# kubeai-project/kubeai

Hardware: AMD Instinct MI355X
Metric: output_tokens_per_s (k6 multi-turn chat) (higher is better)
Workload: dtype fp8; 1 GPU; model=llama-3-8b, global_batch=40, seq_len=8192, parallelism=dp1, prefix_cache=True

## Files before the change

kubeai_amd/csrc/attention_decode.hip:

```cpp
#include <torch/extension.h>

#include <type_traits>

#include "attention_checks.h"
#include "attention_plan.h"
#include "common.h"
#include "dispatch.h"

namespace {

constexpr int kWaves = 2;
constexpr int kBlockThreads = kWaves * WAVE_SIZE;
constexpr int kBS = 16;
typedef __attribute__((ext_vector_type(2))) __bf16 bf16x2v;
constexpr int kPad = 8;

template <int G, typename CT = ushort, int HD = 128, bool CAP = false,
          bool RAW = false>
__launch_bounds__(kBlockThreads) __global__ void paged_decode_kernel(
    ushort* __restrict__ out,
    const ushort* __restrict__ q,
    std::conditional_t<RAW, CT*, const CT*> __restrict__ k_cache,
    std::conditional_t<RAW, CT*, const CT*> __restrict__ v_cache,
    const int32_t* __restrict__ block_tables,
// ... 299 lines not shown
      }

#pragma unroll
      for (int t = tp; t < tp + TOKP; ++t) {
        if (t >= tile_len) break;
        float vv[EPL];
        if constexpr (sizeof(CT) == 2) {
#pragma unroll
          for (int e = 0; e < EPL; e += 2) {
            const uint32_t vr = *reinterpret_cast<const uint32_t*>(
                &v_lds[wave][t][EPL * lane + e]);
            vv[e] = bf16_to_f32((ushort)(vr & 0xffff));
            vv[e + 1] = bf16_to_f32((ushort)(vr >> 16));
          }
        } else {
#pragma unroll
          for (int e = 0; e < EPL; e += 2) {
            const uint32_t vr = *reinterpret_cast<const ushort*>(
                &v_lds[wave][t][EPL * lane + e]);
            const floatx2 vf = __builtin_amdgcn_cvt_pk_f32_bf8(vr, false);
            vv[e] = vf.x;
            vv[e + 1] = vf.y;
          }
        }
#pragma unroll
        for (int g = 0; g < G; ++g) {
          const float pt = __shfl(p[g], (t - tp) * PARTS, 64);
#pragma unroll
          for (int e = 0; e < EPL; ++e)
            o[g][e] = fmaf(pt, vv[e], o[g][e]);
        }
      }
    }

    if (blk_i + kWaves < blk_hi) write_tile();
  }

#pragma unroll
  for (int g = 0; g < G; ++g) {
#pragma unroll
    for (int e = 0; e < EPL; ++e) merge_o[wave][g][EPL * lane + e] = o[g][e];
    if (lane == 0) {
      merge_ml[wave][g][0] = m[g];
      merge_ml[wave][g][1] = l[g];
    }
  }
  __syncthreads();

  for (int g = wave; g < G; g += kWaves) {
    float m_star = -INFINITY;
#pragma unroll
    for (int w = 0; w < kWaves; ++w) m_star = fmaxf(m_star, merge_ml[w][g][0]);
    float l_star = 0.f, oo[EPL];
#pragma unroll
    for (int e = 0; e < EPL; ++e) oo[e] = 0.f;
    if (m_star != -INFINITY) {
#pragma unroll
      for (int w = 0; w < kWaves; ++w) {
        const float c = __expf(merge_ml[w][g][0] - m_star);
        l_star += merge_ml[w][g][1] * c;
#pragma unroll
        for (int e = 0; e < EPL; ++e)
          oo[e] += merge_o[w][g][EPL * lane + e] * c;
      }
    }
    const int head = kh * G + g;
    if (n_splits == 1) {
      const float inv_l = 1.0f / l_star;
      ushort* oh = out + ((int64_t)b * n_q + head) * HD;
#pragma unroll
      for (int e = 0; e < EPL; e += 2) {
        uint32_t packed =
            ((uint32_t)f32_to_bf16(oo[e + 1] * inv_l) << 16) |
            f32_to_bf16(oo[e] * inv_l);
        *reinterpret_cast<uint32_t*>(&oh[EPL * lane + e]) = packed;
      }
    } else {
      float* po = part_o + (((int64_t)b * n_q + head) * n_splits + split) * HD;
#pragma unroll
      for (int e = 0; e < EPL; ++e) po[EPL * lane + e] = oo[e];
      if (lane == 0) {
        float* pm = part_ml + (((int64_t)b * n_q + head) * n_splits + split) * 2;
        pm[0] = m_star;
        pm[1] = l_star;
      }
    }
  }
}

constexpr int kMergeSplitCapLo = 8;
constexpr int kMergeSplitCapHi = 16;

template <int N, int HD, int SCAP>
DEV_INLINE void merge_partials(const float* __restrict__ po,
                               const float* __restrict__ pml,
                               const int n_splits, uint32_t (&packed)[N / 2]) {
  typedef float __attribute__((ext_vector_type(N))) vecN;
  floatx2 ml[SCAP];
  vecN pv[SCAP];
#pragma unroll
  for (int s = 0; s < SCAP; ++s) {
    const int sc = min(s, n_splits - 1);
    ml[s] = *reinterpret_cast<const floatx2*>(pml + 2 * sc);
    pv[s] = *reinterpret_cast<const vecN*>(po + sc * HD);
  }
  __builtin_amdgcn_sched_barrier(0);
  float m_star = -INFINITY;
#pragma unroll
  for (int s = 0; s < SCAP; ++s)
    if (s < n_splits) m_star = fmaxf(m_star, ml[s].x);
  float l_star = 0.f, oo[N];
#pragma unroll
  for (int e = 0; e < N; ++e) oo[e] = 0.f;
#pragma unroll
  for (int s = 0; s < SCAP; ++s) {
    const bool use = s < n_splits && ml[s].x != -INFINITY;
    const float c = __expf(ml[s].x - m_star);
    l_star = use ? l_star + ml[s].y * c : l_star;
#pragma unroll
    for (int e = 0; e < N; ++e) oo[e] = use ? oo[e] + pv[s][e] * c : oo[e];
  }
  const float inv_l = 1.0f / l_star;
#pragma unroll
  for (int e = 0; e < N; e += 2)
    packed[e / 2] = ((uint32_t)f32_to_bf16(oo[e + 1] * inv_l) << 16) |
                    f32_to_bf16(oo[e] * inv_l);
}

template <int HD, int SCAP>
__global__ void decode_merge_kernel(
    ushort* __restrict__ out,
    const float* __restrict__ part_o,
    const float* __restrict__ part_ml,
    const int n_q, const int n_splits, const int64_t n_bh) {
  constexpr int EPL = HD / 64;
  const int64_t bh = (int64_t)blockIdx.x * (blockDim.x / WAVE_SIZE) +
                     threadIdx.x / WAVE_SIZE;
  if (bh >= n_bh) return;
  const int lane = threadIdx.x % WAVE_SIZE;
  uint32_t packed[EPL / 2];
  merge_partials<EPL, HD, SCAP>(part_o + bh * n_splits * HD + EPL * lane,
                                part_ml + bh * n_splits * 2, n_splits, packed);
  ushort* oh = out + bh * HD;
#pragma unroll
  for (int e = 0; e < EPL; e += 2)
    *reinterpret_cast<uint32_t*>(&oh[EPL * lane + e]) = packed[e / 2];
}

constexpr int kMergeVec = 4;
constexpr int kMergeMaxThreads = 1024;
constexpr int kMergeMaxPasses = 2;
constexpr int kMergeRowMax = kMergeMaxThreads * kMergeVec * kMergeMaxPasses;

template <int HD, int kPasses, int SCAP>
__launch_bounds__(kMergeMaxThreads) __global__ void decode_merge_fp8_kernel(
    ushort* __restrict__ out,
    unsigned char* __restrict__ out_fp8,
    float* __restrict__ out_scale,
    const float* __restrict__ part_o,
    const float* __restrict__ part_ml,
    const int n_q, const int n_splits) {
  __shared__ float red[16];
  const int b = blockIdx.x;
  const int row_len = n_q * HD;
  const int nvec = row_len / kMergeVec;
  ushort* orow = out + (int64_t)b * row_len;

  uint32_t packed[kPasses][kMergeVec / 2];
  float amax = 0.f;
#pragma unroll
  for (int it = 0; it < kPasses; ++it) {
    const int i = threadIdx.x + it * blockDim.x;
    if (i < nvec) {
      const int h = (i * kMergeVec) / HD;
      const int col = (i * kMergeVec) % HD;
      const int64_t bh = (int64_t)b * n_q + h;
      merge_partials<kMergeVec, HD, SCAP>(part_o + bh * n_splits * HD + col,
                                          part_ml + bh * n_splits * 2,
                                          n_splits, packed[it]);
      *reinterpret_cast<uint2*>(orow + i * kMergeVec) =
          make_uint2(packed[it][0], packed[it][1]);
#pragma unroll
      for (int e = 0; e < kMergeVec / 2; ++e) {
        const uint32_t pk = packed[it][e];
        amax = fmaxf(amax, fabsf(bf16_to_f32((ushort)(pk & 0xffff))));
        amax = fmaxf(amax, fabsf(bf16_to_f32((ushort)(pk >> 16))));
      }
    }
  }
  const float inv_scale = row_scale_fp8(amax, red, out_scale + b);
  unsigned char* frow = out_fp8 + (int64_t)b * row_len;
#pragma unroll
  for (int it = 0; it < kPasses; ++it) {
    const int i = threadIdx.x + it * blockDim.x;
    if (i < nvec) {
      uchar4 q4;
      const uint32_t p0 = packed[it][0], p1 = packed[it][1];
      q4.x = f32_to_fp8(bf16_to_f32((ushort)(p0 & 0xffff)) * inv_scale);
      q4.y = f32_to_fp8(bf16_to_f32((ushort)(p0 >> 16)) * inv_scale);
      q4.z = f32_to_fp8(bf16_to_f32((ushort)(p1 & 0xffff)) * inv_scale);
      q4.w = f32_to_fp8(bf16_to_f32((ushort)(p1 >> 16)) * inv_scale);
      *reinterpret_cast<uchar4*>(frow + i * kMergeVec) = q4;
    }
  }
}

}

void quant_fp8(torch::Tensor out, torch::Tensor out_scale, torch::Tensor x);

namespace {

struct RawQKV {
  torch::Tensor k, v, positions, cos_sin, slot_mapping;
};

void decode_impl(torch::Tensor out, const c10::optional<torch::Tensor>& out_fp8,
                 const c10::optional<torch::Tensor>& out_scale, torch::Tensor q,
                 torch::Tensor k_cache, torch::Tensor v_cache,
                 torch::Tensor block_tables, torch::Tensor seq_lens,
                 double scale, int64_t window, double softcap,
                 const RawQKV* raw = nullptr) {
  const AttnShape s =
      check_paged_attention(out, q, k_cache, v_cache, block_tables, seq_lens);
  const int B = q.size(0), n_q = s.n_q, n_kv = s.n_kv, hd = s.hd;
  const int max_blocks = s.max_blocks;
  TORCH_CHECK(seq_lens.numel() >= B && block_tables.size(0) >= B);
  const bool want_fp8 = out_fp8.has_value();
  if (want_fp8) {
    TORCH_CHECK(out_scale.has_value());
    check_fp8_out(out, *out_fp8, *out_scale);
  }
  const ushort *k_new = nullptr, *v_new = nullptr;
  const int32_t* positions = nullptr;
  const float* cos_sin = nullptr;
  const int64_t* slot_mapping = nullptr;
  int64_t k_stride = 0, v_stride = 0;
  if (raw != nullptr) {
    const torch::Tensor &k = raw->k, &v = raw->v;
    TORCH_CHECK(k.dim() == 3 && v.dim() == 3);
    TORCH_CHECK(k.scalar_type() == torch::kBFloat16 &&
                v.scalar_type() == torch::kBFloat16);
    TORCH_CHECK(k.size(0) == B && k.size(1) == n_kv && k.size(2) == hd);
    TORCH_CHECK(v.size(0) == B && v.size(1) == n_kv && v.size(2) == hd);
    TORCH_CHECK(k.stride(2) == 1 && k.stride(1) == hd);
    TORCH_CHECK(v.stride(2) == 1 && v.stride(1) == hd);
    TORCH_CHECK(v_cache.sizes() == k_cache.sizes() &&
                v_cache.scalar_type() == k_cache.scalar_type());
    TORCH_CHECK(k_cache.size(3) == hd);
    TORCH_CHECK(raw->positions.scalar_type() == torch::kInt32 &&
                raw->positions.is_contiguous() && raw->positions.numel() >= B);
    TORCH_CHECK(raw->slot_mapping.scalar_type() == torch::kInt64 &&
                raw->slot_mapping.is_contiguous() &&
                raw->slot_mapping.numel() >= B);
    TORCH_CHECK(raw->cos_sin.scalar_type() == torch::kFloat32 &&
                raw->cos_sin.dim() == 2 && raw->cos_sin.size(1) == hd &&
                raw->cos_sin.is_contiguous());
    auto aligned = [](const torch::Tensor& t, int64_t bytes) {
      return reinterpret_cast<uintptr_t>(t.data_ptr()) % bytes == 0 &&
             (t.dim() < 3 || t.stride(0) * t.element_size() % bytes == 0);
    };
    TORCH_CHECK(aligned(q, 8) && aligned(k, 16) && aligned(v, 16) &&
                    aligned(raw->cos_sin, 16) && aligned(k_cache, 16) &&
                    aligned(v_cache, 16),
                "rope_cache_attention_decode: misaligned q/k/v/cos_sin/cache");
    k_new = (const ushort*)k.data_ptr();
    v_new = (const ushort*)v.data_ptr();
    positions = raw->positions.data_ptr<int32_t>();
    cos_sin = raw->cos_sin.data_ptr<float>();
    slot_mapping = raw->slot_mapping.data_ptr<int64_t>();
    k_stride = k.stride(0);
    v_stride = v.stride(0);
  }
  if (B == 0) return;
  const int n_splits = attn_plan::decode_n_splits(B, n_kv, max_blocks);
  torch::Tensor part_o, part_ml;
  float *part_o_ptr = nullptr, *part_ml_ptr = nullptr;
  if (n_splits > 1) {
    auto opts =
        torch::TensorOptions().device(q.device()).dtype(torch::kFloat32);
    part_o = torch::empty({B, n_q, n_splits, (int64_t)hd}, opts);
    part_ml = torch::empty({B, n_q, n_splits, 2}, opts);
    part_o_ptr = part_o.data_ptr<float>();
    part_ml_ptr = part_ml.data_ptr<float>();
  }
  dim3 grid(B * n_kv * n_splits), block(kBlockThreads);
  auto stream = c10::hip::getCurrentHIPStream().stream();
  dispatch_int<1, 2, 4, 5, 6, 8>(s.G, "GQA group size", [&](auto g) {
    dispatch_int<128, 256>(hd, "head dim", [&](auto hdv) {
      dispatch_bool(s.fp8_cache, [&](auto fp8) {
        dispatch_bool(softcap > 0.0, [&](auto cap) {
          dispatch_bool(raw != nullptr, [&](auto rawv) {
            using CT = std::conditional_t<decltype(fp8)::value, unsigned char,
                                          ushort>;
            hipLaunchKernelGGL(
                (paged_decode_kernel<decltype(g)::value, CT,
                                     decltype(hdv)::value, decltype(cap)::value,
                                     decltype(rawv)::value>),
                grid, block, 0, stream, (ushort*)out.data_ptr(),
                (const ushort*)q.data_ptr(), (CT*)k_cache.data_ptr(),
                (CT*)v_cache.data_ptr(), block_tables.data_ptr<int32_t>(),
                seq_lens.data_ptr<int32_t>(), (float)scale, (float)softcap,
                (int)window, n_kv, max_blocks, q.stride(0), n_splits,
                part_o_ptr, part_ml_ptr, k_new, v_new, positions, cos_sin,
                slot_mapping, k_stride, v_stride);
          });
        });
      });
    });
  });
  HIP_CHECK_KERNEL();
  if (n_splits == 1) {
    if (want_fp8) quant_fp8(*out_fp8, *out_scale, out.view({B, -1}));
    return;
  }
  static_assert(kMergeSplitCapHi == 16, "decode_n_splits caps splits at 16");
  TORCH_CHECK(n_splits <= kMergeSplitCapHi);
  const bool fuse_fp8 = want_fp8 && (int64_t)n_q * hd <= kMergeRowMax;
  dispatch_int<128, 256>(hd, "head dim", [&](auto hdv) {
    dispatch_bool(n_splits <= kMergeSplitCapLo, [&](auto lo) {
      constexpr int HD = decltype(hdv)::value;
      constexpr int SCAP =
          decltype(lo)::value ? kMergeSplitCapLo : kMergeSplitCapHi;
      if (fuse_fp8) {
        const int nvec = n_q * hd / kMergeVec;
        const int threads = std::min(
            kMergeMaxThreads, (nvec + WAVE_SIZE - 1) / WAVE_SIZE * WAVE_SIZE);
        dispatch_int<1, 2>(
            (nvec + threads - 1) / threads, "merge pass count", [&](auto p) {
              hipLaunchKernelGGL(
                  (decode_merge_fp8_kernel<HD, decltype(p)::value, SCAP>),
                  dim3(B), dim3(threads), 0, stream, (ushort*)out.data_ptr(),
                  (unsigned char*)out_fp8->data_ptr(),
                  out_scale->data_ptr<float>(), part_o_ptr, part_ml_ptr, n_q,
                  n_splits);
            });
      } else {
        const int64_t n_bh = (int64_t)B * n_q;
        const int wpb = 4;
        hipLaunchKernelGGL((decode_merge_kernel<HD, SCAP>),
                           dim3((uint32_t)((n_bh + wpb - 1) / wpb)),
                           dim3(wpb * WAVE_SIZE), 0, stream,
                           (ushort*)out.data_ptr(), part_o_ptr, part_ml_ptr,
                           n_q, n_splits, n_bh);
      }
    });
  });
  HIP_CHECK_KERNEL();
  if (want_fp8 && !fuse_fp8) quant_fp8(*out_fp8, *out_scale, out.view({B, -1}));
}

}

void paged_attention_decode(torch::Tensor out, torch::Tensor q,
                            torch::Tensor k_cache, torch::Tensor v_cache,
                            torch::Tensor block_tables, torch::Tensor seq_lens,
                            double scale, int64_t window, double softcap) {
  decode_impl(out, c10::nullopt, c10::nullopt, q, k_cache, v_cache,
              block_tables, seq_lens, scale, window, softcap);
}

void paged_attention_decode_fp8(torch::Tensor out, torch::Tensor out_fp8,
                                torch::Tensor out_scale, torch::Tensor q,
                                torch::Tensor k_cache, torch::Tensor v_cache,
                                torch::Tensor block_tables,
                                torch::Tensor seq_lens, double scale,
                                int64_t window, double softcap) {
  decode_impl(out, out_fp8, out_scale, q, k_cache, v_cache, block_tables,
              seq_lens, scale, window, softcap);
}

void rope_cache_attention_decode(
    torch::Tensor out, c10::optional<torch::Tensor> out_fp8,
    c10::optional<torch::Tensor> out_scale, torch::Tensor q, torch::Tensor k,
    torch::Tensor v, torch::Tensor positions, torch::Tensor cos_sin,
    torch::Tensor k_cache, torch::Tensor v_cache, torch::Tensor slot_mapping,
    torch::Tensor block_tables, torch::Tensor seq_lens, double scale,
    int64_t window, double softcap) {
  const RawQKV raw{k, v, positions, cos_sin, slot_mapping};
  decode_impl(out, out_fp8, out_scale, q, k_cache, v_cache, block_tables,
              seq_lens, scale, window, softcap, &raw);
}
```

kubeai_amd/csrc/bindings.cpp:

```cpp
#include <torch/extension.h>

#include <utility>

#include "attention_plan.h"

void rmsnorm(torch::Tensor out, torch::Tensor x, torch::Tensor weight,
             double eps);
void fused_add_rmsnorm(torch::Tensor x, torch::Tensor residual,
                       torch::Tensor weight, double eps);
void rope(torch::Tensor q, torch::Tensor k, torch::Tensor positions,
          torch::Tensor cos_sin);
void rope_and_cache(torch::Tensor q, torch::Tensor k, torch::Tensor v,
                    torch::Tensor positions, torch::Tensor cos_sin,
                    torch::Tensor k_cache, torch::Tensor v_cache,
                    torch::Tensor slot_mapping);
void reshape_and_cache(torch::Tensor k, torch::Tensor v, torch::Tensor k_cache,
                       torch::Tensor v_cache, torch::Tensor slot_mapping);
void paged_attention_decode(torch::Tensor out, torch::Tensor q,
                            torch::Tensor k_cache, torch::Tensor v_cache,
                            torch::Tensor block_tables, torch::Tensor seq_lens,
                            double scale, int64_t window, double softcap);
void paged_attention_decode_fp8(torch::Tensor out, torch::Tensor out_fp8,
                                torch::Tensor out_scale, torch::Tensor q,
                                torch::Tensor k_cache, torch::Tensor v_cache,
                                torch::Tensor block_tables,
                                torch::Tensor seq_lens, double scale,
                                int64_t window, double softcap);
void rope_cache_attention_decode(
    torch::Tensor out, c10::optional<torch::Tensor> out_fp8,
    c10::optional<torch::Tensor> out_scale, torch::Tensor q, torch::Tensor k,
    torch::Tensor v, torch::Tensor positions, torch::Tensor cos_sin,
    torch::Tensor k_cache, torch::Tensor v_cache, torch::Tensor slot_mapping,
    torch::Tensor block_tables, torch::Tensor seq_lens, double scale,
    int64_t window, double softcap);
void paged_attention_prefill(torch::Tensor out, torch::Tensor q,
                             torch::Tensor k_cache, torch::Tensor v_cache,
                             torch::Tensor block_tables,
                             torch::Tensor query_start_loc,
                             torch::Tensor seq_lens, double scale,
                             int64_t window, double softcap);
void silu_and_mul(torch::Tensor out, torch::Tensor x);
void gelu_and_mul(torch::Tensor out, torch::Tensor x);
void skinny_gemm(torch::Tensor y, torch::Tensor x, torch::Tensor w);
void int4_dequant(torch::Tensor out, torch::Tensor qp, torch::Tensor sp,
                  torch::Tensor zp, int64_t N, int64_t K, int64_t group);
void int4_gemm(torch::Tensor y, torch::Tensor x, torch::Tensor qp,
               torch::Tensor sp, torch::Tensor zp, int64_t N, int64_t K,
               int64_t group);
int64_t int4_gemm_tiles(int64_t N, int64_t M);
void greedy_sample(torch::Tensor out, torch::Tensor logits);
void gumbel_sample(torch::Tensor out, torch::Tensor logits,
                   torch::Tensor temperature, torch::Tensor seeds,
                   int64_t step);
void greedy_sample_logprob(torch::Tensor out, torch::Tensor out_logprob,
                           torch::Tensor out_lse, torch::Tensor logits);
void gumbel_sample_logprob(torch::Tensor out, torch::Tensor out_logprob,
                           torch::Tensor out_lse, torch::Tensor logits,
                           torch::Tensor temperature, torch::Tensor seeds,
                           int64_t step);
void token_logprobs(torch::Tensor out_logprob, torch::Tensor out_lse,
                    torch::Tensor logits, torch::Tensor tokens);
void sgmv(torch::Tensor y, torch::Tensor x, torch::Tensor A, torch::Tensor B,
          torch::Tensor idx, double scale);
void register_chwbl(pybind11::module_& m);
pybind11::bytes xgmi_alloc();
void xgmi_connect(int64_t rank, int64_t world,
                  const std::vector<pybind11::bytes>& handles);
void xgmi_fused_allreduce_add_rmsnorm(torch::Tensor x, torch::Tensor residual,
                                      torch::Tensor weight, double eps);
int64_t xgmi_error_count();
int64_t xgmi_max_elems();
void xgmi_shutdown();
void rmsnorm_fp8(torch::Tensor out, torch::Tensor out_scale, torch::Tensor x,
                 torch::Tensor weight, double eps);
void fused_add_rmsnorm_fp8(torch::Tensor out, torch::Tensor out_scale,
                           torch::Tensor x, torch::Tensor residual,
                           torch::Tensor weight, double eps);
void fused_add_rmsnorm_fp8_div(torch::Tensor out, torch::Tensor out_scale,
                               torch::Tensor x, torch::Tensor residual,
                               torch::Tensor weight, double eps,
                               bool write_rows);
void embed_rmsnorm_fp8(torch::Tensor out, torch::Tensor out_scale,
                       torch::Tensor x_out, torch::Tensor ids,
                       torch::Tensor table, torch::Tensor weight, double eps);
void silu_and_mul_fp8(torch::Tensor out, torch::Tensor out_scale,
                      torch::Tensor x);
void quant_fp8(torch::Tensor out, torch::Tensor out_scale, torch::Tensor x);
void quant_fp8_div(torch::Tensor out, torch::Tensor out_scale,
                   torch::Tensor x);
void nucleus_stats(torch::Tensor m, torch::Tensor z, torch::Tensor logits,
                   torch::Tensor temps);
void nucleus_accept(torch::Tensor ok, torch::Tensor logits,
                    torch::Tensor cand, torch::Tensor m, torch::Tensor z,
                    torch::Tensor temps, torch::Tensor top_ps,
                    torch::Tensor top_ks);

static std::pair<int64_t, int64_t> prefill_plan(int64_t Tq, int64_t B,
                                                int64_t n_q, int64_t n_kv,
                                                int64_t hd, int64_t max_blocks,
                                                int64_t window,
                                                double softcap) {
  TORCH_CHECK(n_kv > 0 && n_q % n_kv == 0);
  const attn_plan::PrefillPlan p = attn_plan::prefill_plan(
      Tq, (int)B, (int)n_q, (int)n_kv, (int)hd, (int)max_blocks, window,
      softcap);
  return {p.version, p.waves};
}
static int64_t decode_plan(int64_t B, int64_t n_kv, int64_t max_blocks) {
  return attn_plan::decode_n_splits((int)B, (int)n_kv, (int)max_blocks);
}

PYBIND11_MODULE(TORCH_EXTENSION_NAME, m) {
  m.def("prefill_plan", &prefill_plan,
        "(version, waves per workgroup) paged_attention_prefill launches",
        pybind11::arg("Tq"), pybind11::arg("B"), pybind11::arg("n_q"),
        pybind11::arg("n_kv"), pybind11::arg("hd"),
        pybind11::arg("max_blocks"), pybind11::arg("window") = 0,
        pybind11::arg("softcap") = 0.0);
  m.def("decode_plan", &decode_plan,
        "flash-decoding splits paged_attention_decode launches",
        pybind11::arg("B"), pybind11::arg("n_kv"),
        pybind11::arg("max_blocks"));
  m.def("rmsnorm", &rmsnorm, "RMSNorm (bf16, fp32 accum)");
  m.def("fused_add_rmsnorm", &fused_add_rmsnorm,
        "in-place residual add + RMSNorm");
  m.def("rope", &rope, "NeoX rotary embedding, in-place q/k");
  m.def("rope_and_cache", &rope_and_cache,
        "rotary embedding (in-place q/k) fused with the paged KV cache write");
  m.def("reshape_and_cache", &reshape_and_cache,
        "paged KV cache write (bf16 or fp8 e5m2 cache)");
  m.def("paged_attention_decode", &paged_attention_decode,
        "paged attention, one query token per seq");
  m.def("paged_attention_decode_fp8", &paged_attention_decode_fp8,
        "paged decode attention that also emits the e4m3 row quant of out");
  m.def("rope_cache_attention_decode", &rope_cache_attention_decode,
        "pure-decode step: rotary embedding and KV cache write inside the "
        "decode attention kernel (q, k, v are only read)");
  m.def("paged_attention_prefill", &paged_attention_prefill,
        "paged causal flash attention over cached KV");
  m.def("gelu_and_mul", &gelu_and_mul, "GeGLU tanh-gelu(gate)*up");
  m.def("silu_and_mul", &silu_and_mul, "SwiGLU activation");
  m.def("skinny_gemm", &skinny_gemm, "weight-streaming GEMM for M<=64");
  m.def("int4_dequant", &int4_dequant,
        "packed int4 weight -> bf16 [N, K], bit-equal to Int4Weight.dequant()");
  m.def("int4_gemm", &int4_gemm,
        "fused dequant + GEMM over a packed int4 weight, M <= 64");
  m.def("int4_gemm_tiles", &int4_gemm_tiles,
        "16-column tiles per workgroup int4_gemm launches with",
        pybind11::arg("N"), pybind11::arg("M"));
  m.def("greedy_sample", &greedy_sample, "argmax sampling");
  m.def("gumbel_sample", &gumbel_sample, "temperature sampling (hash RNG)");
  m.def("greedy_sample_logprob", &greedy_sample_logprob,
        "argmax sampling + the token's logprob and the row logsumexp");
  m.def("gumbel_sample_logprob", &gumbel_sample_logprob,
        "temperature sampling + the token's logprob and the row logsumexp");
  m.def("token_logprobs", &token_logprobs,
        "logprob of given tokens and the row logsumexp, one launch");
  m.def("rmsnorm_fp8", &rmsnorm_fp8, "rmsnorm with fused fp8 row quant");
  m.def("fused_add_rmsnorm_fp8", &fused_add_rmsnorm_fp8,
        "residual add + rmsnorm with fused fp8 row quant");
  m.def("fused_add_rmsnorm_fp8_div", &fused_add_rmsnorm_fp8_div,
        "residual add + rmsnorm, then the division-form fp8 row quant of its "
        "bf16 row (lm_head's input)");
  m.def("embed_rmsnorm_fp8", &embed_rmsnorm_fp8,
        "embedding gather + rmsnorm with fused fp8 row quant (layer 0)");
  m.def("silu_and_mul_fp8", &silu_and_mul_fp8, "SwiGLU with fused fp8 quant");
  m.def("quant_fp8", &quant_fp8, "bf16 -> fp8 row quant");
  m.def("quant_fp8_div", &quant_fp8_div,
        "bf16 -> fp8 row quant, division form (Fp8Linear.forward)");
  m.def("nucleus_stats", &nucleus_stats, "per-row softmax max + Z");
  m.def("nucleus_accept", &nucleus_accept,
        "nucleus membership of sampled tokens (mass above < p, rank < k)");
  m.def("xgmi_alloc", &xgmi_alloc, "allocate + export the IPC comm buffer");
  m.def("xgmi_connect", &xgmi_connect, "open peer IPC buffers");
  m.def("xgmi_fused_allreduce_add_rmsnorm", &xgmi_fused_allreduce_add_rmsnorm,
        "one-shot xGMI all-reduce fused with residual add + RMSNorm");
  m.def("xgmi_error_count", &xgmi_error_count, "spin-wait timeout count");
  m.def("xgmi_max_elems", &xgmi_max_elems, "one-shot capacity (bf16 elems)");
  m.def("xgmi_shutdown", &xgmi_shutdown, "free/close comm buffers");
  m.def("sgmv", &sgmv, "segmented gather LoRA apply (one adapter segment)");
  register_chwbl(m);
}
```

kubeai_amd/csrc/rope_cache.hip:

```cpp
#include <torch/extension.h>

#include <type_traits>

#include "common.h"
#include "dispatch.h"

namespace {

DEV_INLINE void store_cache_elem(ushort* p, ushort bf) { *p = bf; }
DEV_INLINE void store_cache_elem(unsigned char* p, ushort bf) {
  *p = f32_to_e5m2(bf16_to_f32(bf));
}

template <typename CT>
__global__ void rope_and_cache_kernel(
    ushort* __restrict__ q,
    ushort* __restrict__ k,
    const ushort* __restrict__ v,
    CT* __restrict__ k_cache,
    CT* __restrict__ v_cache,
    const int32_t* __restrict__ positions,
    const float* __restrict__ cos_sin,
    const int64_t* __restrict__ slot_mapping,
    const int n_q, const int n_kv, const int hd, const int bs,
    const int64_t n_tok, const int64_t q_stride, const int64_t k_stride,
    const int64_t v_stride) {
  const int n_heads = n_q + 2 * n_kv;
  const int64_t flat = (int64_t)blockIdx.x * (blockDim.x / WAVE_SIZE) +
                       threadIdx.x / WAVE_SIZE;
  const int64_t tok = flat / n_heads;
  if (tok >= n_tok) return;
  const int head = (int)(flat % n_heads);
  const int lane = threadIdx.x % WAVE_SIZE;

  if (head >= n_q + n_kv) {
    const int64_t slot = slot_mapping[tok];
    if (slot < 0) return;
    const int h = head - n_q - n_kv;
    const ushort8* src =
        reinterpret_cast<const ushort8*>(v + tok * v_stride + (int64_t)h * hd);
    CT* dst = v_cache + cache_row_offset(slot, bs, n_kv, h, hd);
    const int nvec = hd / 8;
    for (int i = lane; i < nvec; i += WAVE_SIZE) {
      const ushort8 vv = src[i];
      if constexpr (sizeof(CT) == 2) {
        reinterpret_cast<ushort8*>(dst)[i] = vv;
      } else {
        uint64_t vo = 0;
#pragma unroll
        for (int j = 0; j < 8; ++j)
          vo |= (uint64_t)f32_to_e5m2(bf16_to_f32((ushort)vv[j])) << (8 * j);
        reinterpret_cast<uint64_t*>(dst)[i] = vo;
      }
    }
    return;
  }

  const int half = hd / 2;
  const bool is_k = head >= n_q;
  const int pos = positions[tok];
  const float* cs = cos_sin + (int64_t)pos * hd;
  ushort* base = is_k ? k + tok * k_stride + (int64_t)(head - n_q) * hd
                      : q + tok * q_stride + (int64_t)head * hd;
  CT* dst = nullptr;
  if (is_k) {
    const int64_t slot = slot_mapping[tok];
    if (slot >= 0)
      dst = k_cache + cache_row_offset(slot, bs, n_kv, head - n_q, hd);
  }
  for (int i = lane; i < half; i += WAVE_SIZE) {
    const float c = cs[i];
    const float s = cs[half + i];
    const float x1 = bf16_to_f32(base[i]);
    const float x2 = bf16_to_f32(base[half + i]);
    ushort o1, o2;
    rope_rotate_pair(x1, x2, c, s, o1, o2);
    base[i] = o1;
    base[half + i] = o2;
    if (dst != nullptr) {
      store_cache_elem(dst + i, o1);
      store_cache_elem(dst + half + i, o2);
    }
  }
}

}

void rope_and_cache(torch::Tensor q, torch::Tensor k, torch::Tensor v,
                    torch::Tensor positions, torch::Tensor cos_sin,
                    torch::Tensor k_cache, torch::Tensor v_cache,
                    torch::Tensor slot_mapping) {
  TORCH_CHECK(q.dim() == 3 && k.dim() == 3 && v.dim() == 3);
  TORCH_CHECK(q.stride(2) == 1 && q.stride(1) == q.size(2));
  TORCH_CHECK(k.stride(2) == 1 && k.stride(1) == k.size(2));
  TORCH_CHECK(v.stride(2) == 1 && v.stride(1) == v.size(2));
  TORCH_CHECK(q.scalar_type() == torch::kBFloat16 &&
              k.scalar_type() == torch::kBFloat16 &&
              v.scalar_type() == torch::kBFloat16);
  TORCH_CHECK(positions.scalar_type() == torch::kInt32);
  TORCH_CHECK(cos_sin.scalar_type() == torch::kFloat32);
  TORCH_CHECK(slot_mapping.scalar_type() == torch::kInt64);
  TORCH_CHECK(k_cache.is_contiguous() && v_cache.is_contiguous());
  TORCH_CHECK(k_cache.dim() == 4 && v_cache.sizes() == k_cache.sizes());
  const bool fp8_cache = k_cache.scalar_type() == torch::kFloat8_e5m2;
  TORCH_CHECK(fp8_cache || k_cache.scalar_type() == torch::kBFloat16);
  TORCH_CHECK(v_cache.scalar_type() == k_cache.scalar_type());
  const int T = q.size(0);
  const int n_q = q.size(1), n_kv = k.size(1), hd = q.size(2);
  TORCH_CHECK(hd == 128 || hd == 256,
              "rope_and_cache supports head_dim 128 or 256");
  TORCH_CHECK(k.size(0) == T && v.size(0) == T && k.size(2) == hd);
  TORCH_CHECK(v.size(1) == n_kv && v.size(2) == hd);
  TORCH_CHECK(cos_sin.size(1) == hd);
  TORCH_CHECK(k_cache.size(1) == n_kv && k_cache.size(3) == hd);
  TORCH_CHECK(positions.numel() >= T && slot_mapping.numel() >= T);
  TORCH_CHECK(v.stride(0) % 8 == 0 && v.storage_offset() % 8 == 0);
  const int bs = k_cache.size(2);
  if (T == 0) return;
  const int64_t total_waves = (int64_t)T * (n_q + 2 * n_kv);
  const int waves_per_block = 4;
  const int64_t blocks = (total_waves + waves_per_block - 1) / waves_per_block;
  dispatch_bool(fp8_cache, [&](auto fp8) {
    using CT = std::conditional_t<decltype(fp8)::value, unsigned char, ushort>;
    hipLaunchKernelGGL(
        rope_and_cache_kernel<CT>, dim3((uint32_t)blocks),
        dim3(waves_per_block * WAVE_SIZE), 0,
        c10::hip::getCurrentHIPStream().stream(), (ushort*)q.data_ptr(),
        (ushort*)k.data_ptr(), (const ushort*)v.data_ptr(),
        (CT*)k_cache.data_ptr(), (CT*)v_cache.data_ptr(),
        positions.data_ptr<int32_t>(), cos_sin.data_ptr<float>(),
        slot_mapping.data_ptr<int64_t>(), n_q, n_kv, hd, bs, (int64_t)T,
        q.stride(0), k.stride(0), v.stride(0));
  });
  HIP_CHECK_KERNEL();
}
```

kubeai_amd/models/llama.py:

```python
from __future__ import annotations

import math

import torch
import torch.nn as nn
import torch.nn.functional as F

from kubeai_amd import ops
from kubeai_amd.engine.batch import ForwardBatch
from .config import ModelArchConfig


class EngineLinear(nn.Linear):

    def forward(self, x: torch.Tensor) -> torch.Tensor:
        y = ops.linear(x, self.weight)
        if self.bias is not None:
            y = y + self.bias
        return y


def _rms_head(x: torch.Tensor, w: torch.Tensor, eps: float) -> torch.Tensor:
    if x.is_cuda and x.dtype == torch.bfloat16:
        flat = x.contiguous().view(-1, x.shape[-1])
        return ops.rmsnorm(flat, w, eps).view(x.shape)
    xf = x.float()
    xf = xf * torch.rsqrt(xf.pow(2).mean(-1, keepdim=True) + eps)
    return (xf * w.float()).to(x.dtype)


def paged_attention_step(
    q: torch.Tensor,
    k: torch.Tensor,
    v: torch.Tensor,
    fb: ForwardBatch,
    kv_cache: tuple[torch.Tensor, torch.Tensor],
    cos_sin: torch.Tensor,
    *,
    scale: float,
    window: int,
    softcap: float,
    fp8_out: bool,
):
    k_cache, v_cache = kv_cache
    T = q.shape[0]
    out = torch.empty(q.shape, dtype=q.dtype, device=q.device)
    nd = fb.n_decode
    if fb.n_prefill == 0 and nd == T and nd > 0 and q.is_cuda:
        res = ops.rope_cache_attention_decode(
            q,
            k,
            v,
            fb.positions,
            cos_sin,
            k_cache,
            v_cache,
            fb.slot_mapping,
            fb.decode_block_tables,
            fb.decode_seq_lens,
            scale,
            out=out,
            window=window,
            softcap=softcap,
            fp8_out=fp8_out,
        )
        return res[1:] if fp8_out else out.view(T, -1)
    q, k = ops.rope_and_cache(
        q, k, v, fb.positions, cos_sin, k_cache, v_cache, fb.slot_mapping
    )
    if nd > 0:
        ops.paged_attention_decode(
            q[:nd],
            k_cache,
            v_cache,
            fb.decode_block_tables,
            fb.decode_seq_lens,
            scale,
            out=out[:nd],
            window=window,
            softcap=softcap,
        )
    if fb.n_prefill > 0:
        ops.paged_attention_prefill(
            q[nd:],
            k_cache,
            v_cache,
            fb.prefill_block_tables,
            fb.prefill_query_start_loc,
            fb.prefill_seq_lens,
            scale,
            out=out[nd:],
            window=window,
            softcap=softcap,
        )
    attn_flat = out.view(T, -1)
    return ops.quant_fp8(attn_flat) if fp8_out else attn_flat


class Attention(nn.Module):
    def __init__(self, cfg: ModelArchConfig, layer_idx: int):
        super().__init__()
        self.layer_idx = layer_idx
        self.n_q = cfg.num_attention_heads
        self.n_kv = cfg.num_key_value_heads
        self.hd = cfg.head_dim
        if cfg.global_layer_interval > 0:
            self.is_global = (layer_idx + 1) % cfg.global_layer_interval == 0
            use_win = not self.is_global
        else:
            self.is_global = True
            use_win = (
                cfg.sliding_window_pattern != "even" or layer_idx % 2 == 0
            )
        self.window = (cfg.sliding_window or 0) if use_win else 0
        self.qk_norm = cfg.qk_norm
        if cfg.qk_norm:
            self.q_norm = nn.Parameter(torch.ones(cfg.head_dim))
            self.k_norm = nn.Parameter(torch.ones(cfg.head_dim))
        self.norm_eps = cfg.rms_norm_eps
        self.softcap = cfg.attn_logit_softcap or 0.0
        self.scale = (
            cfg.attention_multiplier
            or 1.0 / math.sqrt(cfg.query_pre_attn_scalar or self.hd)
        )
        q_size = self.n_q * self.hd
        kv_size = self.n_kv * self.hd
        self.qkv_proj = EngineLinear(
            cfg.hidden_size, q_size + 2 * kv_size, bias=cfg.attention_bias
        )
        self.o_proj = EngineLinear(q_size, cfg.hidden_size, bias=False)

    def forward(
        self,
        x: torch.Tensor,
        fb: ForwardBatch,
        kv_cache: tuple[torch.Tensor, torch.Tensor],
        cos_sin: torch.Tensor,
    ) -> torch.Tensor:
        fp8_in = isinstance(x, tuple)
        if fp8_in:
            xq, xs = x
            qkv = self.qkv_proj.forward_quantized(xq, xs)
            lm = None
        else:
            qkv = self.qkv_proj(x)
            lm = getattr(self, "_lora_manager", None)
            if lm is not None and lm.active and fb.lora_ids is not None:
                lm.apply(self.layer_idx, "qkv", x, qkv, fb.lora_ids)
        q, k, v = qkv.split(
            [self.n_q * self.hd, self.n_kv * self.hd, self.n_kv * self.hd], dim=-1
        )
        q = q.unflatten(-1, (self.n_q, self.hd))
        k = k.unflatten(-1, (self.n_kv, self.hd))
        v = v.unflatten(-1, (self.n_kv, self.hd))
        if self.qk_norm:
            q = _rms_head(q, self.q_norm, self.norm_eps)
            k = _rms_head(k, self.k_norm, self.norm_eps)
        if isinstance(cos_sin, tuple):
            cos_sin = cos_sin[0] if self.is_global else cos_sin[1]
        attn = paged_attention_step(
            q, k, v, fb, kv_cache, cos_sin, scale=self.scale,
            window=self.window, softcap=self.softcap, fp8_out=fp8_in,
        )
        if fp8_in:
            return self.o_proj.forward_quantized(*attn)
        return self._o_proj_bf16(attn, fb, lm)

    def _o_proj_bf16(self, attn_flat, fb: ForwardBatch, lm) -> torch.Tensor:
        result = self.o_proj(attn_flat)
        if lm is not None and lm.active and fb.lora_ids is not None:
            lm.apply(self.layer_idx, "o", attn_flat, result, fb.lora_ids)
        return result


class MLP(nn.Module):
    def __init__(self, cfg: ModelArchConfig, layer_idx: int | None = None):
        super().__init__()
        self.layer_idx = layer_idx
        self.gate_up_proj = EngineLinear(
            cfg.hidden_size, 2 * cfg.intermediate_size, bias=False
        )
        self.down_proj = EngineLinear(cfg.intermediate_size, cfg.hidden_size, bias=False)
        self.gelu = cfg.hidden_act == "gelu_pytorch_tanh"

    def forward(self, x, fb: ForwardBatch | None = None) -> torch.Tensor:
        if isinstance(x, tuple):
            h = self.gate_up_proj.forward_quantized(*x)
            a8, ascale = ops.silu_and_mul_fp8(h)
            return self.down_proj.forward_quantized(a8, ascale)
        h = self.gate_up_proj(x)
        lm = getattr(self, "_lora_manager", None)
        lora_live = (
            lm is not None and lm.active and fb is not None
            and fb.lora_ids is not None and self.layer_idx is not None
        )
        if lora_live:
            lm.apply(self.layer_idx, "gate_up", x, h, fb.lora_ids)
        a = ops.gelu_and_mul(h) if self.gelu else ops.silu_and_mul(h)
        y = self.down_proj(a)
        if lora_live:
            lm.apply(self.layer_idx, "down", a, y, fb.lora_ids)
        return y


class MoEMLP(nn.Module):

    def __init__(self, cfg: ModelArchConfig):
        super().__init__()
        self.n_experts = cfg.num_local_experts
        self.top_k = cfg.num_experts_per_tok
        self.gate = nn.Linear(cfg.hidden_size, self.n_experts, bias=False)
        self.experts = nn.ModuleList([MLP(cfg) for _ in range(self.n_experts)])

    def forward(self, x: torch.Tensor, fb: ForwardBatch | None = None) -> torch.Tensor:
        T, H = x.shape
        router = F.linear(x.float(), self.gate.weight.float())
        weights, selected = torch.topk(router, self.top_k, dim=-1)
        weights = torch.softmax(weights, dim=-1).to(x.dtype)
        if T <= 256:
            wfull = torch.zeros(T, self.n_experts, dtype=x.dtype,
                                device=x.device)
            wfull.scatter_(1, selected, weights)
# ... 237 lines not shown
```

kubeai_amd/ops/__init__.py:

```python
from __future__ import annotations

import os
from typing import NamedTuple

import torch

from . import ref

_C = None
_C_IMPORT_ERROR: Exception | None = None
try:
    from kubeai_amd import _C
except Exception as e:
    _C_IMPORT_ERROR = e


def have_hip_ext() -> bool:
    return _C is not None


def _require_ext() -> None:
    if _C is None:
        raise RuntimeError(
            "kubeai_amd HIP extension (kubeai_amd._C) is not built but a GPU "
            "tensor reached the ops layer. Build it with "
            "`python setup.py build_ext --inplace` (PYTORCH_ROCM_ARCH=gfx950). "
            f"Original import error: {_C_IMPORT_ERROR!r}"
        )


def rmsnorm(x: torch.Tensor, weight: torch.Tensor, eps: float) -> torch.Tensor:
    if x.is_cuda:
        _require_ext()
        out = torch.empty_like(x)
        _C.rmsnorm(out, x, weight, eps)
        return out
    return ref.rmsnorm(x, weight, eps)


def fused_add_rmsnorm(x, residual, weight, eps: float):
    if x.is_cuda:
        _require_ext()
        _C.fused_add_rmsnorm(x, residual, weight, eps)
        return x, residual
    return ref.fused_add_rmsnorm(x, residual, weight, eps)


def rope(q, k, positions, cos_sin):
    if q.is_cuda:
        _require_ext()
        _C.rope(q, k, positions, cos_sin)
        return q, k
    return ref.rope(q, k, positions, cos_sin)


def reshape_and_cache(k, v, k_cache, v_cache, slot_mapping) -> None:
    if k.is_cuda:
        _require_ext()
        _C.reshape_and_cache(k, v, k_cache, v_cache, slot_mapping)
        return
    ref.reshape_and_cache(k, v, k_cache, v_cache, slot_mapping)


def rope_and_cache(q, k, v, positions, cos_sin, k_cache, v_cache, slot_mapping):
    if q.is_cuda:
        _require_ext()
        _C.rope_and_cache(
            q, k, v, positions, cos_sin, k_cache, v_cache, slot_mapping
        )
        return q, k
    q, k = ref.rope(q, k, positions, cos_sin)
    ref.reshape_and_cache(k, v, k_cache, v_cache, slot_mapping)
    return q, k


def paged_attention_decode(
    q, k_cache, v_cache, block_tables, seq_lens, scale: float, out=None,
    window: int = 0, softcap: float = 0.0, fp8_out: bool = False,
):
    if q.is_cuda:
        _require_ext()
        if out is None:
            out = torch.empty(q.shape, dtype=q.dtype, device=q.device)
        if fp8_out:
            B = q.shape[0]
            o8 = torch.empty(
                (B, q.shape[1] * q.shape[2]), dtype=torch.float8_e4m3fn,
                device=q.device,
            )
            oscale = torch.empty(B, dtype=torch.float32, device=q.device)
            _C.paged_attention_decode_fp8(
                out, o8, oscale, q, k_cache, v_cache, block_tables, seq_lens,
                scale, window, softcap
            )
            return out, o8, oscale
        _C.paged_attention_decode(
            out, q, k_cache, v_cache, block_tables, seq_lens, scale, window,
            softcap
        )
        return out
    res = ref.paged_attention_decode(
        q, k_cache, v_cache, block_tables, seq_lens, scale, window=window,
        softcap=softcap,
    )
    if out is not None:
        out.copy_(res)
        res = out
    if fp8_out:
        o8, oscale = ref.quant_fp8(res.reshape(res.shape[0], -1))
        return res, o8, oscale
    return res


def decode_rope_fused() -> bool:
    return os.environ.get("KUBEAI_DECODE_ROPE_FUSED", "1") != "0"


def rope_cache_attention_decode(
    q, k, v, positions, cos_sin, k_cache, v_cache, slot_mapping,
    block_tables, seq_lens, scale: float, out=None, window: int = 0,
    softcap: float = 0.0, fp8_out: bool = False,
):
    if q.is_cuda and decode_rope_fused():
        _require_ext()
        if out is None:
            out = torch.empty(q.shape, dtype=q.dtype, device=q.device)
        o8 = oscale = None
        if fp8_out:
            o8, oscale = _empty_fp8_rows(
                (q.shape[0], q.shape[1] * q.shape[2]), q.device
            )
        _C.rope_cache_attention_decode(
            out, o8, oscale, q, k, v, positions, cos_sin, k_cache, v_cache,
            slot_mapping, block_tables, seq_lens, scale, window, softcap
        )
        return (out, o8, oscale) if fp8_out else out
    if not q.is_cuda:
        res = ref.rope_cache_attention_decode(
            q, k, v, positions, cos_sin, k_cache, v_cache, slot_mapping,
            block_tables, seq_lens, scale, window=window, softcap=softcap,
        )
        if out is not None:
            out.copy_(res)
            res = out
        if fp8_out:
            o8, oscale = ref.quant_fp8(res.reshape(res.shape[0], -1))
            return res, o8, oscale
        return res
    qr, _ = rope_and_cache(
        q, k, v, positions, cos_sin, k_cache, v_cache, slot_mapping
    )
    return paged_attention_decode(
        qr, k_cache, v_cache, block_tables, seq_lens, scale, out=out,
        window=window, softcap=softcap, fp8_out=fp8_out,
    )


def paged_attention_prefill(
    q, k_cache, v_cache, block_tables, query_start_loc, seq_lens, scale: float,
    out=None, window: int = 0, softcap: float = 0.0,
):
    if q.is_cuda:
        _require_ext()
        if out is None:
            out = torch.empty(q.shape, dtype=q.dtype, device=q.device)
        _C.paged_attention_prefill(
            out, q, k_cache, v_cache, block_tables, query_start_loc, seq_lens,
            scale, window, softcap
        )
        return out
    res = ref.paged_attention_prefill(
        q, k_cache, v_cache, block_tables, query_start_loc, seq_lens, scale,
        window=window, softcap=softcap,
    )
    if out is not None:
        out.copy_(res)
        return out
    return res


def silu_and_mul(x):
    if x.is_cuda:
        _require_ext()
        T, two_i = x.shape
        out = torch.empty((T, two_i // 2), dtype=x.dtype, device=x.device)
        _C.silu_and_mul(out, x)
        return out
    return ref.silu_and_mul(x)


def gelu_and_mul(x):
    if x.is_cuda:
        _require_ext()
        T, two_i = x.shape
        out = torch.empty((T, two_i // 2), dtype=x.dtype, device=x.device)
        _C.gelu_and_mul(out, x)
        return out
    return ref.gelu_and_mul(x)


_USE_SKINNY = os.environ.get("KUBEAI_SKINNY_GEMM", "0") == "1"


def linear(x, weight):
    if (
        _USE_SKINNY
        and x.is_cuda
        and x.dtype == torch.bfloat16
        and x.dim() == 2
        and 1 <= x.shape[0] <= 64
        and weight.shape[1] % 64 == 0
        and weight.shape[0] % 64 == 0
        and x.is_contiguous()
        and weight.is_contiguous()
    ):
        _require_ext()
        y = torch.empty(
            (x.shape[0], weight.shape[0]), dtype=x.dtype, device=x.device
        )
        _C.skinny_gemm(y, x, weight)
        return y
    return torch.nn.functional.linear(x, weight)



INT4_M_FUSED = int(os.environ.get("KUBEAI_INT4_M_FUSED", "64"))

_INT4_WORKSPACE: dict = {}


def int4_reserve_workspace(device, numel: int) -> None:
    device = torch.device(device)
    ws = _INT4_WORKSPACE.get(device)
    if ws is None or ws.numel() < numel:
        _INT4_WORKSPACE[device] = torch.empty(
            numel, dtype=torch.bfloat16, device=device
        )


def int4_dequant(w, out=None):
    if not w.qp.is_cuda:
        res = w.dequant()
        if out is not None:
            out.copy_(res)
            return out
        return res
    _require_ext()
    if out is None:
        out = torch.empty((w.N, w.K), dtype=torch.bfloat16, device=w.qp.device)
    _C.int4_dequant(out, w.qp, w.sp, w.zp, w.N, w.K, w.group)
    return out


def int4_linear(x, w):
    if not x.is_cuda:
        return torch.nn.functional.linear(x, w.dequant())
    _require_ext()
    if x.dim() != 2:
        return int4_linear(x.reshape(-1, x.shape[-1]), w).view(*x.shape[:-1], w.N)
    M = x.shape[0]
    if 1 <= M <= min(INT4_M_FUSED, 64):
        if x.stride(1) != 1 or x.stride(0) % 8 or x.data_ptr() % 16:
            x = x.contiguous()
        y = torch.empty((M, w.N), dtype=torch.bfloat16, device=x.device)
# ... 224 lines not shown
```

Before: 7789 tok/s.

## Fuse mixed-batch fp8 quant into decode merge and vectorize rope_and_cache

```diff
diff --git a/kubeai_amd/csrc/attention_decode.hip b/kubeai_amd/csrc/attention_decode.hip
--- a/kubeai_amd/csrc/attention_decode.hip
+++ b/kubeai_amd/csrc/attention_decode.hip
@@ -475,14 +475,15 @@
 constexpr int kMergeMaxPasses = 2;
 constexpr int kMergeRowMax = kMergeMaxThreads * kMergeVec * kMergeMaxPasses;
 
-template <int HD, int kPasses, int SCAP>
+template <int HD, int kPasses, int SCAP, bool kTail = false>
 __launch_bounds__(kMergeMaxThreads) __global__ void decode_merge_fp8_kernel(
     ushort* __restrict__ out,
     unsigned char* __restrict__ out_fp8,
     float* __restrict__ out_scale,
     const float* __restrict__ part_o,
     const float* __restrict__ part_ml,
-    const int n_q, const int n_splits) {
+    const int n_q, const int n_splits,
+    const int n_merge = 0) {
   __shared__ float red[16];
   const int b = blockIdx.x;
   const int row_len = n_q * HD;
@@ -495,14 +496,20 @@
   for (int it = 0; it < kPasses; ++it) {
     const int i = threadIdx.x + it * blockDim.x;
     if (i < nvec) {
-      const int h = (i * kMergeVec) / HD;
-      const int col = (i * kMergeVec) % HD;
-      const int64_t bh = (int64_t)b * n_q + h;
-      merge_partials<kMergeVec, HD, SCAP>(part_o + bh * n_splits * HD + col,
-                                          part_ml + bh * n_splits * 2,
-                                          n_splits, packed[it]);
-      *reinterpret_cast<uint2*>(orow + i * kMergeVec) =
-          make_uint2(packed[it][0], packed[it][1]);
+      if (kTail && b >= n_merge) {
+        const uint2 t = *reinterpret_cast<const uint2*>(orow + i * kMergeVec);
+        packed[it][0] = t.x;
+        packed[it][1] = t.y;
+      } else {
+        const int h = (i * kMergeVec) / HD;
+        const int col = (i * kMergeVec) % HD;
+        const int64_t bh = (int64_t)b * n_q + h;
+        merge_partials<kMergeVec, HD, SCAP>(part_o + bh * n_splits * HD + col,
+                                            part_ml + bh * n_splits * 2,
+                                            n_splits, packed[it]);
+        *reinterpret_cast<uint2*>(orow + i * kMergeVec) =
+            make_uint2(packed[it][0], packed[it][1]);
+      }
 #pragma unroll
       for (int e = 0; e < kMergeVec / 2; ++e) {
         const uint32_t pk = packed[it][e];
@@ -543,13 +550,16 @@
                  torch::Tensor k_cache, torch::Tensor v_cache,
                  torch::Tensor block_tables, torch::Tensor seq_lens,
                  double scale, int64_t window, double softcap,
-                 const RawQKV* raw = nullptr) {
+                 const RawQKV* raw = nullptr, const int64_t n_tail = 0) {
   const AttnShape s =
       check_paged_attention(out, q, k_cache, v_cache, block_tables, seq_lens);
   const int B = q.size(0), n_q = s.n_q, n_kv = s.n_kv, hd = s.hd;
   const int max_blocks = s.max_blocks;
   TORCH_CHECK(seq_lens.numel() >= B && block_tables.size(0) >= B);
   const bool want_fp8 = out_fp8.has_value();
+  TORCH_CHECK(n_tail >= 0 && (n_tail == 0 || want_fp8));
+  const int64_t rows = B + n_tail;
+  TORCH_CHECK(out.numel() == rows * n_q * hd, "out must have ", rows, " rows");
   if (want_fp8) {
     TORCH_CHECK(out_scale.has_value());
     check_fp8_out(out, *out_fp8, *out_scale);
@@ -595,7 +605,10 @@
     k_stride = k.stride(0);
     v_stride = v.stride(0);
   }
-  if (B == 0) return;
+  if (B == 0) {
+    if (n_tail > 0) quant_fp8(*out_fp8, *out_scale, out.view({rows, -1}));
+    return;
+  }
   const int n_splits = attn_plan::decode_n_splits(B, n_kv, max_blocks);
   torch::Tensor part_o, part_ml;
   float *part_o_ptr = nullptr, *part_ml_ptr = nullptr;
@@ -634,7 +647,7 @@
   });
   HIP_CHECK_KERNEL();
   if (n_splits == 1) {
-    if (want_fp8) quant_fp8(*out_fp8, *out_scale, out.view({B, -1}));
+    if (want_fp8) quant_fp8(*out_fp8, *out_scale, out.view({rows, -1}));
     return;
   }
   static_assert(kMergeSplitCapHi == 16, "decode_n_splits caps splits at 16");
@@ -651,12 +664,16 @@
             kMergeMaxThreads, (nvec + WAVE_SIZE - 1) / WAVE_SIZE * WAVE_SIZE);
         dispatch_int<1, 2>(
             (nvec + threads - 1) / threads, "merge pass count", [&](auto p) {
-              hipLaunchKernelGGL(
-                  (decode_merge_fp8_kernel<HD, decltype(p)::value, SCAP>),
-                  dim3(B), dim3(threads), 0, stream, (ushort*)out.data_ptr(),
-                  (unsigned char*)out_fp8->data_ptr(),
-                  out_scale->data_ptr<float>(), part_o_ptr, part_ml_ptr, n_q,
-                  n_splits);
+              dispatch_bool(n_tail > 0, [&](auto tail) {
+                hipLaunchKernelGGL(
+                    (decode_merge_fp8_kernel<HD, decltype(p)::value, SCAP,
+                                             decltype(tail)::value>),
+                    dim3((uint32_t)rows), dim3(threads), 0, stream,
+                    (ushort*)out.data_ptr(),
+                    (unsigned char*)out_fp8->data_ptr(),
+                    out_scale->data_ptr<float>(), part_o_ptr, part_ml_ptr, n_q,
+                    n_splits, B);
+              });
             });
       } else {
         const int64_t n_bh = (int64_t)B * n_q;
@@ -670,7 +687,8 @@
     });
   });
   HIP_CHECK_KERNEL();
-  if (want_fp8 && !fuse_fp8) quant_fp8(*out_fp8, *out_scale, out.view({B, -1}));
+  if (want_fp8 && !fuse_fp8)
+    quant_fp8(*out_fp8, *out_scale, out.view({rows, -1}));
 }
 
 }
@@ -691,6 +709,18 @@
                                 int64_t window, double softcap) {
   decode_impl(out, out_fp8, out_scale, q, k_cache, v_cache, block_tables,
               seq_lens, scale, window, softcap);
+}
+
+void paged_attention_decode_fp8_tail(torch::Tensor out, torch::Tensor out_fp8,
+                                     torch::Tensor out_scale, torch::Tensor q,
+                                     torch::Tensor k_cache,
+                                     torch::Tensor v_cache,
+                                     torch::Tensor block_tables,
+                                     torch::Tensor seq_lens, double scale,
+                                     int64_t window, double softcap) {
+  decode_impl(out, out_fp8, out_scale, q, k_cache, v_cache, block_tables,
+              seq_lens, scale, window, softcap, nullptr,
+              out.size(0) - q.size(0));
 }
 
 void rope_cache_attention_decode(
diff --git a/kubeai_amd/csrc/bindings.cpp b/kubeai_amd/csrc/bindings.cpp
--- a/kubeai_amd/csrc/bindings.cpp
+++ b/kubeai_amd/csrc/bindings.cpp
@@ -14,6 +14,9 @@
                     torch::Tensor positions, torch::Tensor cos_sin,
                     torch::Tensor k_cache, torch::Tensor v_cache,
                     torch::Tensor slot_mapping);
+bool rope_and_cache_vec_ok(torch::Tensor q, torch::Tensor k, torch::Tensor v,
+                           torch::Tensor cos_sin, torch::Tensor k_cache,
+                           torch::Tensor v_cache);
 void reshape_and_cache(torch::Tensor k, torch::Tensor v, torch::Tensor k_cache,
                        torch::Tensor v_cache, torch::Tensor slot_mapping);
 void paged_attention_decode(torch::Tensor out, torch::Tensor q,
@@ -26,6 +29,13 @@
                                 torch::Tensor block_tables,
                                 torch::Tensor seq_lens, double scale,
                                 int64_t window, double softcap);
+void paged_attention_decode_fp8_tail(torch::Tensor out, torch::Tensor out_fp8,
+                                     torch::Tensor out_scale, torch::Tensor q,
+                                     torch::Tensor k_cache,
+                                     torch::Tensor v_cache,
+                                     torch::Tensor block_tables,
+                                     torch::Tensor seq_lens, double scale,
+                                     int64_t window, double softcap);
 void rope_cache_attention_decode(
     torch::Tensor out, c10::optional<torch::Tensor> out_fp8,
     c10::optional<torch::Tensor> out_scale, torch::Tensor q, torch::Tensor k,
@@ -127,12 +137,18 @@
   m.def("rope", &rope, "NeoX rotary embedding, in-place q/k");
   m.def("rope_and_cache", &rope_and_cache,
         "rotary embedding (in-place q/k) fused with the paged KV cache write");
+  m.def("rope_cache_vec_ok", &rope_and_cache_vec_ok,
+        "whether rope_and_cache runs its 16-byte vector kernel on these "
+        "tensors (the 2-byte fallback otherwise)");
   m.def("reshape_and_cache", &reshape_and_cache,
         "paged KV cache write (bf16 or fp8 e5m2 cache)");
   m.def("paged_attention_decode", &paged_attention_decode,
         "paged attention, one query token per seq");
   m.def("paged_attention_decode_fp8", &paged_attention_decode_fp8,
         "paged decode attention that also emits the e4m3 row quant of out");
+  m.def("paged_attention_decode_fp8_tail", &paged_attention_decode_fp8_tail,
+        "paged decode attention into the first rows of out, and the e4m3 row "
+        "quant of all of out (the tail rows are already written)");
   m.def("rope_cache_attention_decode", &rope_cache_attention_decode,
         "pure-decode step: rotary embedding and KV cache write inside the "
         "decode attention kernel (q, k, v are only read)");
diff --git a/kubeai_amd/csrc/rope_cache.hip b/kubeai_amd/csrc/rope_cache.hip
--- a/kubeai_amd/csrc/rope_cache.hip
+++ b/kubeai_amd/csrc/rope_cache.hip
@@ -84,6 +84,97 @@
   }
 }
 
+DEV_INLINE void store_cache_vec(ushort* p, const ushort8 v) {
+  *reinterpret_cast<ushort8*>(p) = v;
+}
+DEV_INLINE void store_cache_vec(unsigned char* p, const ushort8 v) {
+  uint64_t vo = 0;
+#pragma unroll
+  for (int j = 0; j < 8; ++j)
+    vo |= (uint64_t)f32_to_e5m2(bf16_to_f32((ushort)v[j])) << (8 * j);
+  *reinterpret_cast<uint64_t*>(p) = vo;
+}
+
+template <typename CT, int HD>
+__global__ void rope_and_cache_vec_kernel(
+    ushort* __restrict__ q,
+    ushort* __restrict__ k,
+    const ushort* __restrict__ v,
+    CT* __restrict__ k_cache,
+    CT* __restrict__ v_cache,
+    const int32_t* __restrict__ positions,
+    const float* __restrict__ cos_sin,
+    const int64_t* __restrict__ slot_mapping,
+    const int n_q, const int n_kv, const int bs, const int64_t q_stride,
+    const int64_t k_stride, const int64_t v_stride) {
+  constexpr int HALF = HD / 2;
+  constexpr int LPH = HALF / 8;
+  const int64_t tok = blockIdx.x;
+  const int in_tok = blockIdx.y * blockDim.x + threadIdx.x;
+  if (in_tok >= (n_q + 2 * n_kv) * LPH) return;
+  const int head = in_tok / LPH;
+  const int e0 = (in_tok % LPH) * 8;
+  const int64_t slot = slot_mapping[tok];
+
+  if (head >= n_q + n_kv) {
+    if (slot < 0) return;
+    const int h = head - n_q - n_kv;
+    const ushort* src = v + tok * v_stride + (int64_t)h * HD + e0;
+    const ushort8 lo = *reinterpret_cast<const ushort8*>(src);
+    const ushort8 hi = *reinterpret_cast<const ushort8*>(src + HALF);
+    CT* dst = v_cache + cache_row_offset(slot, bs, n_kv, h, HD) + e0;
+    store_cache_vec(dst, lo);
+    store_cache_vec(dst + HALF, hi);
+    return;
+  }
+
+  const bool is_k = head >= n_q;
+  const int pos = positions[tok];
+  const float* cs = cos_sin + (int64_t)pos * HD + e0;
+  ushort* base = (is_k ? k + tok * k_stride + (int64_t)(head - n_q) * HD
+                       : q + tok * q_stride + (int64_t)head * HD) +
+                 e0;
+  const ushort8 x1 = *reinterpret_cast<const ushort8*>(base);
+  const ushort8 x2 = *reinterpret_cast<const ushort8*>(base + HALF);
+  float4_t c[2], sn[2];
+#pragma unroll
+  for (int h = 0; h < 2; ++h) {
+    c[h] = *reinterpret_cast<const float4_t*>(cs + 4 * h);
+    sn[h] = *reinterpret_cast<const float4_t*>(cs + HALF + 4 * h);
+  }
+  ushort8 r1, r2;
+#pragma unroll
+  for (int e = 0; e < 8; ++e) {
+    ushort o1, o2;
+    rope_rotate_pair(bf16_to_f32(x1[e]), bf16_to_f32(x2[e]), c[e / 4][e % 4],
+                     sn[e / 4][e % 4], o1, o2);
+    r1[e] = o1;
+    r2[e] = o2;
+  }
+  *reinterpret_cast<ushort8*>(base) = r1;
+  *reinterpret_cast<ushort8*>(base + HALF) = r2;
+  if (is_k && slot >= 0) {
+    CT* dst = k_cache + cache_row_offset(slot, bs, n_kv, head - n_q, HD) + e0;
+    store_cache_vec(dst, r1);
+    store_cache_vec(dst + HALF, r2);
+  }
+}
+
+}
+
+bool rope_and_cache_vec_ok(torch::Tensor q, torch::Tensor k, torch::Tensor v,
+                           torch::Tensor cos_sin, torch::Tensor k_cache,
+                           torch::Tensor v_cache) {
+  auto base_aligned = [](const torch::Tensor& t) {
+    return reinterpret_cast<uintptr_t>(t.data_ptr()) % 16 == 0;
+  };
+  auto rows_aligned = [&](const torch::Tensor& t) {
+    return t.stride(0) % 8 == 0 && t.storage_offset() % 8 == 0 &&
+           base_aligned(t);
+  };
+  return rows_aligned(q) && rows_aligned(k) && rows_aligned(v) &&
+         cos_sin.is_contiguous() && base_aligned(cos_sin) &&
+         base_aligned(k_cache) && base_aligned(v_cache);
 }
 
 void rope_and_cache(torch::Tensor q, torch::Tensor k, torch::Tensor v,
@@ -117,6 +208,28 @@
   TORCH_CHECK(v.stride(0) % 8 == 0 && v.storage_offset() % 8 == 0);
   const int bs = k_cache.size(2);
   if (T == 0) return;
+  auto stream = c10::hip::getCurrentHIPStream().stream();
+  if (rope_and_cache_vec_ok(q, k, v, cos_sin, k_cache, v_cache)) {
+    const int threads = 128;
+    const int per_tok = (n_q + 2 * n_kv) * (hd / 16);
+    const dim3 grid((uint32_t)T, (uint32_t)((per_tok + threads - 1) / threads));
+    dispatch_bool(fp8_cache, [&](auto fp8) {
+      dispatch_int<128, 256>(hd, "head dim", [&](auto hdv) {
+        using CT =
+            std::conditional_t<decltype(fp8)::value, unsigned char, ushort>;
+        hipLaunchKernelGGL(
+            (rope_and_cache_vec_kernel<CT, decltype(hdv)::value>),
+            grid, dim3(threads), 0, stream, (ushort*)q.data_ptr(),
+            (ushort*)k.data_ptr(), (const ushort*)v.data_ptr(),
+            (CT*)k_cache.data_ptr(), (CT*)v_cache.data_ptr(),
+            positions.data_ptr<int32_t>(), cos_sin.data_ptr<float>(),
+            slot_mapping.data_ptr<int64_t>(), n_q, n_kv, bs, q.stride(0),
+            k.stride(0), v.stride(0));
+      });
+    });
+    HIP_CHECK_KERNEL();
+    return;
+  }
   const int64_t total_waves = (int64_t)T * (n_q + 2 * n_kv);
   const int waves_per_block = 4;
   const int64_t blocks = (total_waves + waves_per_block - 1) / waves_per_block;
@@ -124,8 +237,7 @@
     using CT = std::conditional_t<decltype(fp8)::value, unsigned char, ushort>;
     hipLaunchKernelGGL(
         rope_and_cache_kernel<CT>, dim3((uint32_t)blocks),
-        dim3(waves_per_block * WAVE_SIZE), 0,
-        c10::hip::getCurrentHIPStream().stream(), (ushort*)q.data_ptr(),
+        dim3(waves_per_block * WAVE_SIZE), 0, stream, (ushort*)q.data_ptr(),
         (ushort*)k.data_ptr(), (const ushort*)v.data_ptr(),
         (CT*)k_cache.data_ptr(), (CT*)v_cache.data_ptr(),
         positions.data_ptr<int32_t>(), cos_sin.data_ptr<float>(),
diff --git a/kubeai_amd/models/llama.py b/kubeai_amd/models/llama.py
--- a/kubeai_amd/models/llama.py
+++ b/kubeai_amd/models/llama.py
@@ -68,6 +68,30 @@
     q, k = ops.rope_and_cache(
         q, k, v, fb.positions, cos_sin, k_cache, v_cache, fb.slot_mapping
     )
+    if fp8_out and nd > 0 and fb.n_prefill > 0 and ops.mixed_epilogue_fused():
+        ops.paged_attention_prefill(
+            q[nd:],
+            k_cache,
+            v_cache,
+            fb.prefill_block_tables,
+            fb.prefill_query_start_loc,
+            fb.prefill_seq_lens,
+            scale,
+            out=out[nd:],
+            window=window,
+            softcap=softcap,
+        )
+        return ops.paged_attention_decode_fp8_tail(
+            q[:nd],
+            k_cache,
+            v_cache,
+            fb.decode_block_tables,
+            fb.decode_seq_lens,
+            scale,
+            out=out,
+            window=window,
+            softcap=softcap,
+        )
     if nd > 0:
         ops.paged_attention_decode(
             q[:nd],
diff --git a/kubeai_amd/ops/__init__.py b/kubeai_amd/ops/__init__.py
--- a/kubeai_amd/ops/__init__.py
+++ b/kubeai_amd/ops/__init__.py
@@ -110,6 +110,34 @@
         o8, oscale = ref.quant_fp8(res.reshape(res.shape[0], -1))
         return res, o8, oscale
     return res
+
+
+def mixed_epilogue_fused() -> bool:
+    return os.environ.get("KUBEAI_MIXED_EPILOGUE_FUSED", "1") != "0"
+
+
+def paged_attention_decode_fp8_tail(
+    q, k_cache, v_cache, block_tables, seq_lens, scale: float, out,
+    window: int = 0, softcap: float = 0.0,
+):
+    T = out.shape[0]
+    nd = q.shape[0]
+    if q.is_cuda:
+        _require_ext()
+        o8, oscale = _empty_fp8_rows((T, q.shape[1] * q.shape[2]), q.device)
+        _C.paged_attention_decode_fp8_tail(
+            out, o8, oscale, q, k_cache, v_cache, block_tables, seq_lens,
+            scale, window, softcap
+        )
+        return o8, oscale
+    if nd > 0:
+        out[:nd].copy_(
+            ref.paged_attention_decode(
+                q, k_cache, v_cache, block_tables, seq_lens, scale,
+                window=window, softcap=softcap,
+            )
+        )
+    return ref.quant_fp8(out.reshape(T, -1))
 
 
 def decode_rope_fused() -> bool:
```

Measured after the change: 7797 tok/s, median of 2. No clear change (+0.1%).
